# argumentcomputer/lurk-beta

Measured on NVIDIA H100. Metric: Lurk iterations proved/sec (fib rc=100, Nova IVC), higher is better.
Workload: dtype u32x8 (254-bit Montgomery integers)

## Files before the change

### lurk-beta_b200/csrc/curve.cuh

```cuda
#pragma once
#include "field.cuh"

namespace lurk {

template <class F>
struct Affine {
    F x, y;
    LURK_HD bool is_identity() const { return x.is_zero() && y.is_zero(); }
};

template <class F>
LURK_HD F mul_sub_mul(const F &a, const F &b, const F &c, const F &d) {
    WideAcc<typename F::Params> acc;
    acc.clear();
    acc.mul_acc(a, b);
    acc.mul_acc(c.neg(), d);
    return acc.reduce();
}

template <class F>
struct XYZZ {
    F x, y, zz, zzz;

    LURK_HD static XYZZ identity() { XYZZ r; r.x = F::zero(); r.y = F::zero(); r.zz = F::zero(); r.zzz = F::zero(); return r; }
// ... 51 lines not shown
        F ppp = p * pp;
        F q_ = x * pp;
        F x3 = r.sqr() - ppp - q_.dbl();
        y = mul_sub_mul(r, q_ - x3, y, ppp);
        x = x3;
        zz = zz * pp;
        zzz = zzz * ppp;
    }
    LURK_HD void add(const XYZZ &o) {
        if (o.is_identity()) return;
        if (is_identity()) { *this = o; return; }
        F u1 = x * o.zz;
        F u2 = o.x * zz;
        F s1 = y * o.zzz;
        F s2 = o.y * zzz;
        F p = u2 - u1;
        F r = s2 - s1;
        if (p.is_zero()) {
            if (r.is_zero()) *this = dbl(); else *this = identity();
            return;
        }
        F pp = p.sqr();
        F ppp = p * pp;
        F q_ = u1 * pp;
        F x3 = r.sqr() - ppp - q_.dbl();
        y = mul_sub_mul(r, q_ - x3, s1, ppp);
        x = x3;
        zz = zz * o.zz * pp;
        zzz = zzz * o.zzz * ppp;
    }
    LURK_HD Affine<F> to_affine() const {
        Affine<F> a;
        if (is_identity()) { a.x = F::zero(); a.y = F::zero(); return a; }
        F zi = zzz.inv();
        F zz_inv = (zi * zz).sqr();
        a.x = x * zz_inv;
        a.y = y * zi;
        return a;
    }
    LURK_HD XYZZ mul_u32(uint32_t k) const {
        XYZZ acc = identity();
        for (int b = 31; b >= 0; b--) {
            acc = acc.dbl();
            if ((k >> b) & 1) acc.add(*this);
        }
        return acc;
    }
};

struct CurveBn254G1 {
    using Base = Fe<Bn254Fq>; using Scalar = Fe<Bn254Fr>;
    static constexpr int ID = 0; static constexpr bool GEN_X_NEG1 = false;
    LURK_HD static constexpr uint32_t GEN_Y(int i) { constexpr uint32_t t[8] = {2, 0, 0, 0, 0, 0, 0, 0}; return t[i]; }
};
struct CurveGrumpkin {
    using Base = Fe<Bn254Fr>; using Scalar = Fe<Bn254Fq>;
    static constexpr int ID = 1; static constexpr bool GEN_X_NEG1 = false;
    LURK_HD static constexpr uint32_t GEN_Y(int i) {
        constexpr uint32_t t[8] = {0x823f272cu, 0x833fc48du, 0xf1181294u, 0x2d270d45u, 0x06a45d63u, 0xcf135e75u, 0x00000002u, 0x00000000u};
        return t[i];
    }
};
struct CurvePallas {
    using Base = Fe<PallasFp>; using Scalar = Fe<PallasFq>;
    static constexpr int ID = 2; static constexpr bool GEN_X_NEG1 = true;
    LURK_HD static constexpr uint32_t GEN_Y(int i) { constexpr uint32_t t[8] = {2, 0, 0, 0, 0, 0, 0, 0}; return t[i]; }
};
// ... 19 lines not shown
```

### lurk-beta_b200/csrc/field.cuh

```cuda
#pragma once
#include <cstdint>
#include <cstring>

#if defined(__CUDACC__)
#define LURK_HD __host__ __device__ __forceinline__
#define LURK_D __device__ __forceinline__
#else
#define LURK_HD inline
#define LURK_D inline
#endif

#include "field_consts.cuh"

namespace lurk {

namespace cc {
#if defined(__CUDA_ARCH__)
LURK_D uint32_t add_cc(uint32_t a, uint32_t b) { uint32_t r; asm volatile("add.cc.u32 %0, %1, %2;" : "=r"(r) : "r"(a), "r"(b)); return r; }
LURK_D uint32_t addc_cc(uint32_t a, uint32_t b) { uint32_t r; asm volatile("addc.cc.u32 %0, %1, %2;" : "=r"(r) : "r"(a), "r"(b)); return r; }
LURK_D uint32_t addc(uint32_t a, uint32_t b) { uint32_t r; asm volatile("addc.u32 %0, %1, %2;" : "=r"(r) : "r"(a), "r"(b)); return r; }
LURK_D uint32_t sub_cc(uint32_t a, uint32_t b) { uint32_t r; asm volatile("sub.cc.u32 %0, %1, %2;" : "=r"(r) : "r"(a), "r"(b)); return r; }
LURK_D uint32_t subc_cc(uint32_t a, uint32_t b) { uint32_t r; asm volatile("subc.cc.u32 %0, %1, %2;" : "=r"(r) : "r"(a), "r"(b)); return r; }
LURK_D uint32_t subc(uint32_t a, uint32_t b) { uint32_t r; asm volatile("subc.u32 %0, %1, %2;" : "=r"(r) : "r"(a), "r"(b)); return r; }
LURK_D uint32_t mul_lo(uint32_t a, uint32_t b) { uint32_t r; asm volatile("mul.lo.u32 %0, %1, %2;" : "=r"(r) : "r"(a), "r"(b)); return r; }
// ... 202 lines not shown
        uint32_t u[8], w[8];
        Fe x1 = zero(), x2 = zero();
        x1.v[0] = 1;
#pragma unroll
        for (int i = 0; i < 8; i++) { u[i] = v[i]; w[i] = P::MOD(i); }
        auto is_one = [](const uint32_t *a) { uint32_t o = a[0] ^ 1u; for (int i = 1; i < 8; i++) o |= a[i]; return o == 0; };
        auto shr1 = [](uint32_t *a) { for (int i = 0; i < 7; i++) a[i] = (a[i] >> 1) | (a[i + 1] << 31); a[7] >>= 1; };
        auto halve = [&](Fe &x) {
            if (x.v[0] & 1u) {
                x.v[0] = cc::add_cc(x.v[0], P::MOD(0));
                for (int i = 1; i < 7; i++) x.v[i] = cc::addc_cc(x.v[i], P::MOD(i));
                x.v[7] = cc::addc(x.v[7], P::MOD(7));
            }
            shr1(x.v);
        };
        auto sub_raw = [](uint32_t *a, const uint32_t *b) {
            a[0] = cc::sub_cc(a[0], b[0]);
            for (int i = 1; i < 8; i++) a[i] = cc::subc_cc(a[i], b[i]);
            return cc::subc(0, 0);
        };
        auto geq = [](const uint32_t *a, const uint32_t *b) {
            for (int i = 7; i >= 0; i--) { if (a[i] > b[i]) return true; if (a[i] < b[i]) return false; }
            return true;
        };
        while (!is_one(u) && !is_one(w)) {
            while (!(u[0] & 1u)) { shr1(u); halve(x1); }
            while (!(w[0] & 1u)) { shr1(w); halve(x2); }
            if (geq(u, w)) { sub_raw(u, w); x1 = x1 - x2; }
            else { sub_raw(w, u); x2 = x2 - x1; }
        }
        const Fe r3 = rr() * rr();
        return (is_one(u) ? x1 : x2) * r3;
    }
    LURK_HD Fe inv() const {
        uint32_t e[8];
        e[0] = cc::sub_cc(P::MOD(0), 2);
#pragma unroll
        for (int i = 1; i < 8; i++) e[i] = cc::subc_cc(P::MOD(i), 0);
        return pow_raw(e);
    }
};

template <class P, int ROUNDS>
LURK_HD Fe<P> redc17(uint32_t *t) {
    uint32_t r[9];
#pragma unroll
    for (int k = 0; k < 9; k++) r[k] = 0;
#pragma unroll
    for (int i = 0; i < 8; i++) {
        uint32_t mi = t[i] * P::M0;
        Fe<P>::template cmad_mod<0>(t + i, mi);
        r[i] = cc::addc(r[i], 0);
        Fe<P>::template cmad_mod<1>(t + i + 1, mi);
        r[i + 1] = cc::addc(r[i + 1], 0);
    }
    t[8] = cc::add_cc(t[8], r[0]);
#pragma unroll
    for (int k = 1; k < 8; k++) t[8 + k] = cc::addc_cc(t[8 + k], r[k]);
    t[16] = cc::addc(t[16], r[8]);
#pragma unroll
    for (int round = 0; round < ROUNDS; round++) {
        uint32_t d[9];
        d[0] = cc::sub_cc(t[8], P::MOD(0));
#pragma unroll
        for (int k = 1; k < 8; k++) d[k] = cc::subc_cc(t[8 + k], P::MOD(k));
        d[8] = cc::subc_cc(t[16], 0);
// ... 94 lines not shown
```

### lurk-beta_b200/csrc/foldctx_impl.cuh

```cuda
#pragma once
#include "msm_impl.cuh"
#include "poseidon_api.h"
#include "spmv3.cuh"

#include <memory>
#include <string>

namespace lurk {

static constexpr int FOLD_MAX_WORLD = 16;
static constexpr int FOLD_MAX_DEPTH = 4;
static constexpr int FOLD_MAX_SPANS = 4;
static constexpr int FOLD_RO_RATE = 24;
static constexpr int FOLD_W_WINDOW = 17;
static constexpr int FOLD_T_WINDOW = 16;

template <class F>
__global__ void __launch_bounds__(256) cross_term_dev_kernel(const F *__restrict__ az1, const F *__restrict__ bz1, const F *__restrict__ cz1,
                                                             const F *__restrict__ az2, const F *__restrict__ bz2, const F *__restrict__ cz2,
                                                             const F *__restrict__ u1p, const F *__restrict__ u2p, size_t n, F *__restrict__ t) {
    const F u1 = load_fe<F>(u1p), u2 = load_fe<F>(u2p);
    for (size_t i = (size_t)blockIdx.x * blockDim.x + threadIdx.x; i < n; i += (size_t)gridDim.x * blockDim.x) {
        WideAcc<typename F::Params> acc;
        acc.clear();
// ... 227 lines not shown
            const unsigned long long *flag = &a.peers[a.rank]->slot[parity][lane].flag;
            const unsigned long long t0 = globaltimer_ns();
            while (ld_acquire_sys(flag) < seq) {
                if (globaltimer_ns() - t0 > 4000000000ull) { sh_status = 1; break; }
                __nanosleep(200);
            }
        }
        __syncwarp();
        if (lane < a.world) {
            const XchgSlot<Fb> *src = &a.peers[a.rank]->slot[parity][lane];
            const uint4 *q = reinterpret_cast<const uint4 *>(warp == 0 ? &src->w : &src->t);
            uint4 wd[8];
#pragma unroll
            for (int k = 0; k < 8; k++) wd[k] = ld_volatile_u4(q + k);
            const uint32_t *u = reinterpret_cast<const uint32_t *>(wd);
#pragma unroll
            for (int k = 0; k < 8; k++) { pt.x.v[k] = u[k]; pt.y.v[k] = u[8 + k]; pt.zz.v[k] = u[16 + k]; pt.zzz.v[k] = u[24 + k]; }
        }
        int span = 1;
        while (span < a.world) span <<= 1;
#pragma unroll 1
        for (int d = span >> 1; d > 0; d >>= 1) {
            const Pt p2 = shfl_xor_xyzz(pt, d);
            pt.add(p2);
        }
    }
    if (lane == 0) sh_pt[warp] = pt;
    __syncthreads();

    if (tid == 0) {
        const Pt pw = sh_pt[0], pc = sh_pt[1];
        const bool iw = pw.is_identity(), ic = pc.is_identity();
        const Fb zw = iw ? Fb::one() : pw.zzz, zc = ic ? Fb::one() : pc.zzz;
        const Fb inv = (zw * zc).inv_vartime();
        const Fb iwz = inv * zc, icz = inv * zw;
        Fb x = Fb::zero(), y = Fb::zero();
        if (!iw) { const Fb zz_inv = (iwz * pw.zz).sqr(); x = pw.x * zz_inv; y = pw.y * iwz; }
        sh_aff[0] = x; sh_aff[1] = y;
        x = Fb::zero(); y = Fb::zero();
        if (!ic) { const Fb zz_inv = (icz * pc.zz).sqr(); x = pc.x * zz_inv; y = pc.y * icz; }
        sh_aff[2] = x; sh_aff[3] = y;
        sh_inf[0] = iw; sh_inf[1] = ic;
        a.rec->cw_x = sh_aff[0]; a.rec->cw_y = sh_aff[1]; a.rec->ct_x = sh_aff[2]; a.rec->ct_y = sh_aff[3];
        a.rec->cw_inf = iw; a.rec->ct_inf = ic;
        a.rec->status = sh_status;
        a.rec->seq = seq;
    }
    __syncthreads();
    if (a.mode != FOLD_MODE_FOLD || warp != 0) return;

    Fb s = Fb::zero();
    if (lane == 0) s = a.io_tag;
    else if (lane <= a.n_absorb) {
        switch (a.kind[lane - 1]) {
            case FOLD_RO_W_X: s = sh_aff[0]; break;
            case FOLD_RO_W_Y: s = sh_aff[1]; break;
            case FOLD_RO_W_INF: s = sh_inf[0] ? Fb::one() : Fb::zero(); break;
            case FOLD_RO_T_X: s = sh_aff[2]; break;
            case FOLD_RO_T_Y: s = sh_aff[3]; break;
            case FOLD_RO_T_INF: s = sh_inf[1] ? Fb::one() : Fb::zero(); break;
            default: s = load_fe<Fb>(a.step_consts + (lane - 1)); break;
        }
    }
    s = ro_permute_warp<Fb>(a.ro_consts, a.L, s, lane);
    if (lane == 1) {
        a.rec->hash = s;
        const Fb h = s.to_canonical();
// ... 17 lines not shown
__global__ void __launch_bounds__(64) fold_commitments_kernel(XYZZ<typename C::Base> *run_w, XYZZ<typename C::Base> *run_e,
                                                              FoldRecord<typename C::Base, typename C::Scalar> *rec, int init) {
    using Fb = typename C::Base;
    using Fs = typename C::Scalar;
    using Pt = XYZZ<Fb>;
    const int which = threadIdx.x >> 5;
    if (threadIdx.x & 31) return;
    Affine<Fb> q;
    q.x = which == 0 ? rec->cw_x : rec->ct_x;
    q.y = which == 0 ? rec->cw_y : rec->ct_y;
    Pt *run = which == 0 ? run_w : run_e;
    Pt acc;
    if (init) {
        acc = which == 0 ? Pt::from_affine(q) : Pt::identity();
    } else {
        const Fs k = rec->r.to_canonical();
        acc = Pt::identity();
        int top = 255;
        while (top >= 0 && !((k.v[top >> 5] >> (top & 31)) & 1u)) top--;
#pragma unroll 1
        for (int b = top; b >= 0; b--) {
            acc = acc.dbl();
            if ((k.v[b >> 5] >> (b & 31)) & 1u) acc.add_affine(q);
        }
        Pt cur = *run;
        cur.add(acc);
        acc = cur;
    }
    *run = acc;
    Affine<Fb> af;
    af.x = Fb::zero();
    af.y = Fb::zero();
    if (!acc.is_identity()) {
        const Fb zi = acc.zzz.inv_vartime();
        const Fb zz_inv = (zi * acc.zz).sqr();
        af.x = acc.x * zz_inv;
        af.y = acc.y * zi;
    }
    if (which == 0) { rec->uw_x = af.x; rec->uw_y = af.y; rec->uw_inf = acc.is_identity(); }
    else { rec->ue_x = af.x; rec->ue_y = af.y; rec->ue_inf = acc.is_identity(); }
}

struct FoldSpan { uint64_t first, row_elems, stride, rows; };

struct FoldSlotBatch {
    int arity = 0;
    size_t count = 0;
    DevBuf d_offsets;
    DevBuf d_pre[FOLD_MAX_DEPTH];
    void *h_pre[FOLD_MAX_DEPTH] = {nullptr, nullptr, nullptr, nullptr};
    size_t bytes() const { return count * (size_t)(arity ? arity : 1) * 32; }
};

struct FoldConfigHost {
    int curve_id = 0, depth = 2, world = 1, rank = 0;
    uint64_t n_w = 0, n_x = 0, n_rows = 0;
    int latency_sms = 0;
};

struct FoldResultHost {
    uint8_t comm_w[96], comm_t[96], r[32], run_comm_w[96], run_comm_e[96], hash[32];
    int status;
    unsigned long long seq;
};

struct FoldCtxBase {
    virtual ~FoldCtxBase() {}
// ... 29 lines not shown
```

### lurk-beta_b200/csrc/msm_impl.cuh

```cuda
#pragma once
#include "common.cuh"

#include <algorithm>
#include <atomic>
#include <mutex>
#include <thread>

namespace lurk {

static constexpr uint32_t KEY_NONE = 0xffffffffu;

struct MsmPlan {
    int c = 0;
    int nwin = 0;
    uint32_t nb = 0;
    uint32_t total_buckets = 0;
    uint32_t seg = 0;
    uint32_t t1 = 0;
    bool fixed = false;
    uint32_t rwin = 0, K = 0, G = 0, nq = 0, SL = 0, slice = 0;
};
static constexpr uint32_t MSM_MAX_RESULT_POINTS = 512;

inline int fixed_base_window(size_t key_n) {
// ... 83 lines not shown
}

static __global__ void __launch_bounds__(1024) msm_scan_tile_sums_kernel(const uint32_t *__restrict__ counts, uint32_t len, uint32_t *__restrict__ tile_sums) {
    const uint32_t base = blockIdx.x * SCAN_TILE + threadIdx.x * 4;
    uint32_t sum = 0;
#pragma unroll
    for (int k = 0; k < 4; k++) if (base + k < len) sum += counts[base + k];
    uint32_t total;
    block_exclusive_scan_1024(sum, &total);
    if (threadIdx.x == 0) tile_sums[blockIdx.x] = total;
}
static __global__ void __launch_bounds__(1024) msm_scan_tiles_kernel(const uint32_t *__restrict__ tile_sums, uint32_t ntiles, uint32_t *__restrict__ tile_offsets) {
    const uint32_t base = threadIdx.x * 4;
    uint32_t v[4], sum = 0;
#pragma unroll
    for (int k = 0; k < 4; k++) { v[k] = base + k < ntiles ? tile_sums[base + k] : 0; sum += v[k]; }
    uint32_t total;
    uint32_t run = block_exclusive_scan_1024(sum, &total);
#pragma unroll
    for (int k = 0; k < 4; k++) { if (base + k < ntiles) tile_offsets[base + k] = run; run += v[k]; }
    if (threadIdx.x == 0) tile_offsets[ntiles] = total;
}
struct BucketPartials { uint32_t first, count; };
__host__ __device__ __forceinline__ BucketPartials bucket_partials(uint32_t lo, uint32_t hi, uint32_t seg) {
    BucketPartials r{lo / seg + 1, 0};
    if (hi >= lo + 2) {
        const uint32_t last = (hi - 1) / seg;
        if (last >= r.first) r.count = last - r.first + 1;
    }
    return r;
}
static constexpr uint32_t MSM_LONG_PARTIALS = 16;

static __global__ void __launch_bounds__(1024) msm_scan_apply_kernel(const uint32_t *__restrict__ counts, uint32_t len, const uint32_t *__restrict__ tile_offsets,
                                                              uint32_t ntiles, uint32_t *__restrict__ offsets, uint32_t seg = 0,
                                                              uint32_t *long_list = nullptr) {
    const uint32_t base = blockIdx.x * SCAN_TILE + threadIdx.x * 4;
    uint32_t v[4], sum = 0;
#pragma unroll
    for (int k = 0; k < 4; k++) { v[k] = base + k < len ? counts[base + k] : 0; sum += v[k]; }
    uint32_t run = tile_offsets[blockIdx.x] + block_exclusive_scan_1024(sum, nullptr);
#pragma unroll
    for (int k = 0; k < 4; k++) {
        if (base + k < len) {
            offsets[base + k] = run;
            if (long_list && bucket_partials(run, run + v[k], seg).count > MSM_LONG_PARTIALS) long_list[atomicAdd(long_list - 1, 1u)] = base + k;
        }
        run += v[k];
    }
    if (blockIdx.x == 0 && threadIdx.x == 0) offsets[len] = tile_offsets[ntiles];
}

template <class Fs>
__global__ void __launch_bounds__(256) msm_scatter_kernel(const Fs *__restrict__ scalars, const Fs *__restrict__ sub, size_t n, int fmt, int c, int nwin,
                                                          uint32_t key_stride, uint32_t base_stride, const uint32_t *__restrict__ offsets,
                                                          uint32_t *__restrict__ cursor, uint32_t *__restrict__ sorted) {
    size_t i = (size_t)blockIdx.x * blockDim.x + threadIdx.x;
    const bool live = i < n;
    Fs k = Fs::zero();
    if (live) {
        k = load_fe<Fs>(scalars + i);
        if (sub) k = k - load_fe<Fs>(sub + i);
        if (fmt == LURK_FMT_MONTGOMERY) k = k.to_canonical();
    }
    uint32_t carry = 0;
    const uint32_t half = 1u << (c - 1);
    const uint32_t lane = threadIdx.x & 31;
    for (int w = 0; w < nwin; w++) {
        uint32_t raw = window_bits(k.v, w * c, c) + carry;
// ... 102 lines not shown
    PairIn<Fb> r;
    r.p1 = pair_load<Fb, FIRST>(sorted, pts, in);
    r.kind = 0;
    r.p2 = r.p1;
    if (in + 1 < run_end) {
        r.p2 = pair_load<Fb, FIRST>(sorted, pts, in + 1);
        if (r.p1.is_identity()) { r.p1 = r.p2; }
        else if (r.p2.is_identity()) {}
        else if (r.p1.x == r.p2.x) r.kind = (r.p1.y == r.p2.y && !r.p1.y.is_zero()) ? 2 : 3;
        else r.kind = 1;
    }
    return r;
}
template <class Fb>
__device__ __forceinline__ Fb pair_denominator(const PairIn<Fb> &in) {
    if (in.kind == 1) return in.p2.x - in.p1.x;
    if (in.kind == 2) return in.p1.y.dbl();
    return Fb::one();
}

template <class Fb>
__device__ __forceinline__ Fb warp_batch_inverse(const Fb &v) {
    const int lane = threadIdx.x & 31;
    Fb pre = v, suf = v;
#pragma unroll 1
    for (int d = 1; d < 32; d <<= 1) {
        Fb a, b;
#pragma unroll
        for (int i = 0; i < 8; i++) { a.v[i] = __shfl_up_sync(0xffffffffu, pre.v[i], d); b.v[i] = __shfl_down_sync(0xffffffffu, suf.v[i], d); }
        if (lane >= d) pre = pre * a;
        if (lane + d < 32) suf = suf * b;
    }
    Fb inv = Fb::zero();
    if (lane == 31) inv = pre.inv_vartime();
    Fb ep, es, r;
#pragma unroll
    for (int i = 0; i < 8; i++) {
        ep.v[i] = __shfl_up_sync(0xffffffffu, pre.v[i], 1);
        es.v[i] = __shfl_down_sync(0xffffffffu, suf.v[i], 1);
        r.v[i] = __shfl_sync(0xffffffffu, inv.v[i], 31);
    }
    if (lane > 0) r = r * ep;
    if (lane < 31) r = r * es;
    return r;
}

template <class Fb, bool FIRST>
__global__ void __launch_bounds__(128) msm_pair_kernel(const uint32_t *__restrict__ offs_in, const uint32_t *__restrict__ offs_out, uint32_t nbuckets,
                                                       const uint32_t *__restrict__ sorted, const Affine<Fb> *__restrict__ pts_in,
                                                       Affine<Fb> *__restrict__ pts_out) {
    const uint32_t total = offs_out[nbuckets];
    const uint64_t gtid = (uint64_t)blockIdx.x * blockDim.x + threadIdx.x;
    if ((gtid & ~31ull) * PAIR_B >= total) return;
    const uint64_t start64 = gtid * PAIR_B;
    const bool active = start64 < total;
    const uint32_t start = active ? (uint32_t)start64 : 0, end = active ? (uint32_t)min((uint64_t)total, start64 + PAIR_B) : 0;
    uint32_t k = 0;
    if (active) {
        uint32_t lo = 0, hi = nbuckets;
        while (hi - lo > 1) { const uint32_t mid = (lo + hi) >> 1; if (offs_out[mid] <= start) lo = mid; else hi = mid; }
        k = lo;
    }
    Fb pref[PAIR_B];
    Fb run = Fb::one();
    for (uint32_t q = start; q < end; q++) {
        while (offs_out[k + 1] <= q) k++;
        const uint32_t in = offs_in[k] + 2 * (q - offs_out[k]);
        const PairIn<Fb> pi = pair_fetch<Fb, FIRST>(sorted, pts_in, in, offs_in[k + 1]);
        run = run * pair_denominator(pi);
        pref[q - start] = run;
    }
    Fb inv = warp_batch_inverse(run);
    for (uint32_t q = end; q-- > start;) {
        while (offs_out[k] > q) k--;
        const uint32_t in = offs_in[k] + 2 * (q - offs_out[k]);
        const PairIn<Fb> pi = pair_fetch<Fb, FIRST>(sorted, pts_in, in, offs_in[k + 1]);
        const uint32_t j = q - start;
        const Fb den = pair_denominator(pi);
        const Fb inv_d = j ? inv * pref[j - 1] : inv;
        inv = inv * den;
        Affine<Fb> o = pi.p1;
        if (pi.kind == 3) { o.x = Fb::zero(); o.y = Fb::zero(); }
        else if (pi.kind) {
            Fb num;
            if (pi.kind == 1) num = pi.p2.y - pi.p1.y;
            else { const Fb xx = pi.p1.x.sqr(); num = xx.dbl() + xx; }
            const Fb lam = num * inv_d;
            const Fb x3 = lam.sqr() - pi.p1.x - pi.p2.x;
            o.y = lam * (pi.p1.x - x3) - pi.p1.y;
            o.x = x3;
        }
        store_fe(&pts_out[q].x, o.x);
        store_fe(&pts_out[q].y, o.y);
    }
}

static constexpr uint32_t MSM_MERGE_THREADS = 64, MSM_MERGE_LONG_THREADS = 256;
template <class Fb>
__global__ void __launch_bounds__(MSM_MERGE_THREADS) msm_merge_kernel(const uint32_t *__restrict__ offsets, uint32_t nbuckets, uint32_t seg,
                                                                      const XYZZ<Fb> *__restrict__ ppt, XYZZ<Fb> *__restrict__ bucket_acc) {
    const uint32_t b = blockIdx.x * MSM_MERGE_THREADS + threadIdx.x;
    if (b >= nbuckets) return;
    const uint32_t lo = offsets[b], hi = offsets[b + 1];
    const BucketPartials bp = bucket_partials(lo, hi, seg);
    if (bp.count > MSM_LONG_PARTIALS) return;
    XYZZ<Fb> acc = XYZZ<Fb>::identity();
    if (hi > lo) acc = load_xyzz(bucket_acc + b);
    for (uint32_t i = 0; i < bp.count; i++) acc.add(load_xyzz(ppt + bp.first + i));
    store_xyzz(bucket_acc + b, acc);
}

template <class Fb>
__global__ void __launch_bounds__(MSM_MERGE_LONG_THREADS) msm_merge_long_kernel(const uint32_t *__restrict__ offsets, uint32_t seg,
                                                                                const XYZZ<Fb> *__restrict__ ppt, const uint32_t *__restrict__ long_list,
                                                                                XYZZ<Fb> *__restrict__ bucket_acc) {
    __shared__ XYZZ<Fb> sm[MSM_MERGE_LONG_THREADS];
    const uint32_t tid = threadIdx.x, nlong = long_list[-1];
    for (uint32_t i = blockIdx.x; i < nlong; i += gridDim.x) {
        const uint32_t b = long_list[i];
        const BucketPartials bp = bucket_partials(offsets[b], offsets[b + 1], seg);
        XYZZ<Fb> acc = XYZZ<Fb>::identity();
        if (tid == 0) acc = load_xyzz(bucket_acc + b);
        for (uint32_t j = tid; j < bp.count; j += MSM_MERGE_LONG_THREADS) acc.add(load_xyzz(ppt + bp.first + j));
        sm[tid] = acc;
        __syncthreads();
        for (uint32_t stride = MSM_MERGE_LONG_THREADS / 2; stride > 0; stride >>= 1) {
            if (tid < stride) { XYZZ<Fb> x = sm[tid]; x.add(sm[tid + stride]); sm[tid] = x; }
            __syncthreads();
        }
        if (tid == 0) store_xyzz(bucket_acc + b, sm[0]);
        __syncthreads();
    }
}


template <class Fb>
__global__ void __launch_bounds__(128) msm_chunk_kernel(const XYZZ<Fb> *__restrict__ bucket_acc, uint32_t K, uint32_t nchunks_total,
                                                        XYZZ<Fb> *__restrict__ tri_out, XYZZ<Fb> *__restrict__ run_out) {
    const uint32_t g = blockIdx.x * blockDim.x + threadIdx.x;
    if (g >= nchunks_total) return;
    const XYZZ<Fb> *B = bucket_acc + (size_t)g * K;
    XYZZ<Fb> run = XYZZ<Fb>::identity(), tri = XYZZ<Fb>::identity();
    for (int b = (int)K - 1; b >= 0; b--) {
        run.add(load_xyzz(B + b));
        tri.add(run);
    }
    store_xyzz(tri_out + g, tri);
    store_xyzz(run_out + g, run);
}

// ... 165 lines not shown
    cudaEvent_t ev0 = nullptr, ev1 = nullptr;
    float last_accumulate_ms = 0.f;
    unsigned last_launches = 0;
    bool pending = false;
    int pending_fmt = 0, pending_c = 0, pending_nwin = 0;
    bool pending_fixed = false;
    uint32_t pending_nq = 0, pending_K = 0;
    cudaEvent_t done = nullptr;
    cudaStream_t tiny_stream = nullptr;
    const void *d_sub = nullptr;
    const void *d_offset = nullptr;
    cudaEvent_t ev_fork = nullptr, ev_join = nullptr;
};

namespace lurk {

template <class Fb>
void point_to_bytes(const XYZZ<Fb> &p, int fmt, uint8_t out[96]) {
    memset(out, 0, 96);
    if (p.is_identity()) return;
    Affine<Fb> a = p.to_affine();
    Fb one = Fb::one();
    if (fmt == LURK_FMT_CANONICAL) { a.x = a.x.to_canonical(); a.y = a.y.to_canonical(); one = one.to_canonical(); }
    memcpy(out, a.x.v, 32); memcpy(out + 32, a.y.v, 32); memcpy(out + 64, one.v, 32);
}

inline int ctx_check_device(const lurk_msm_ctx *ctx) {
    int dev = -1;
    LURK_CUDA_TRY(cudaGetDevice(&dev));
    if (dev != ctx->device) { set_error("context belongs to device %d but device %d is current", ctx->device, dev); return LURK_ERR_ARG; }
    return LURK_OK;
}

template <class C>
int msm_launch(lurk_msm_ctx *ctx, const void *d_scalars, size_t n, int fmt, cudaStream_t s, bool readback) {
    using Fb = typename C::Base;
    using Fs = typename C::Scalar;
    using Pt = XYZZ<Fb>;
    if (ctx->pending) { set_error("a launch is already pending on this context (call lurk_msm_ctx_finish)"); return LURK_ERR_ARG; }
    LURK_TRY(ctx_check_device(ctx));
    if (!ctx->done) LURK_CUDA_TRY(cudaEventCreateWithFlags(&ctx->done, cudaEventDisableTiming));
    ctx->pending_fmt = fmt;
    ctx->pending_nwin = 0;
    MsmScratch &S = ctx->scratch;
    if (S.result.bytes < sizeof(Pt)) LURK_TRY(S.result.alloc(sizeof(Pt)));
    if (n == 0) {
        if (readback) ctx->pending = true;
        else LURK_CUDA_TRY(cudaMemsetAsync(S.result.p, 0, sizeof(Pt), s));
        return LURK_OK;
    }
    const bool table_pays = !readback || n * (size_t)(Fs::Params::NBITS / std::max(ctx->fixed_c, 1) + 1) >= ((size_t)8 << (std::max(ctx->fixed_c, 1) - 1));
    const bool fixed = ctx->d_table != nullptr && table_pays;
    if (!readback && !fixed) { set_error("device-resident results need the fixed-base table (lurk_msm_ctx_precompute)"); return LURK_ERR_ARG; }
    MsmPlan P = make_plan(n, Fs::Params::NBITS, fixed ? ctx->fixed_c : 0);
    if ((uint64_t)n * (uint64_t)P.nwin >= (1ull << 32)) { set_error("%zu scalars exceed one launch (shard the commitment key)", n); return LURK_ERR_ARG; }
    const uint32_t TB = P.total_buckets;
    const uint32_t ntiles = (TB + SCAN_TILE - 1) / SCAN_TILE;
    const size_t cap = n * (size_t)P.nwin;
    int rounds = 0;
    {
        static const int forced = [] { const char *e = getenv("LURK_MSM_PAIR_ROUNDS"); return e ? atoi(e) : -1; }();
        const size_t avg = cap / TB;
        if (forced >= 0) rounds = forced;
        else if (n >= 8192) rounds = avg >= 12 ? MSM_PAIR_ROUNDS_LONG : (avg >= 5 ? MSM_PAIR_ROUNDS_SHORT : 0);
        if (rounds > 4) rounds = 4;
    }
    size_t cap_final = cap;
    for (int r = 0; r < rounds; r++) cap_final = cap_final / 2 + TB + 1;
    const uint32_t t1 = rounds ? (uint32_t)((cap_final + P.seg - 1) / P.seg) : P.t1;
    const uint32_t t1_alloc = std::max(t1, P.t1);
    const uint32_t max_long = t1 / (MSM_LONG_PARTIALS + 1) + 1;
    {
        auto ensure = [](DevBuf &b, size_t bytes) { return b.bytes >= bytes ? LURK_OK : b.alloc(bytes); };
        LURK_TRY(ensure(S.counts, (((size_t)TB + 1) * 2 + 1 + max_long) * sizeof(uint32_t)));
        LURK_TRY(ensure(S.offsets, ((size_t)TB + 1) * sizeof(uint32_t)));
        LURK_TRY(ensure(S.tiles, ((size_t)ntiles + 1) * 2 * sizeof(uint32_t)));
        LURK_TRY(ensure(S.sorted, n * (size_t)P.nwin * sizeof(uint32_t)));
        LURK_TRY(ensure(S.buckets, (size_t)TB * sizeof(Pt)));
        LURK_TRY(ensure(S.ppt, (size_t)t1_alloc * sizeof(Pt)));
        const size_t nchunks_all = (size_t)P.rwin * P.G;
        LURK_TRY(ensure(S.chunks, nchunks_all * sizeof(Pt)));
        LURK_TRY(ensure(S.chunk_sums, nchunks_all * sizeof(Pt)));
        LURK_TRY(ensure(S.slices, (size_t)P.rwin * P.nq * P.SL * sizeof(Pt)));
        LURK_TRY(ensure(S.wins, MSM_MAX_RESULT_POINTS * sizeof(Pt)));
        if (!S.h_wins) LURK_CUDA_TRY(cudaMallocHost(&S.h_wins, MSM_MAX_RESULT_POINTS * sizeof(Pt)));
    }
    if (ntiles > 4096) { set_error("bucket table too large for the scan"); return LURK_ERR_ARG; }
    uint32_t *counts = S.counts.as<uint32_t>();
    uint32_t *cursor = counts + (TB + 1);
    uint32_t *offsets = S.offsets.as<uint32_t>();
    uint32_t *tile_sums = S.tiles.as<uint32_t>(), *tile_offsets = tile_sums + (ntiles + 1);
    uint32_t *sorted = S.sorted.as<uint32_t>();
    uint32_t *long_list = cursor + (TB + 1) + 1;
    Pt *buckets = S.buckets.as<Pt>();

    LURK_CUDA_TRY(cudaMemsetAsync(counts, 0, (((size_t)TB + 1) * 2 + 1) * sizeof(uint32_t), s));
    const unsigned gs = (unsigned)((n + 255) / 256);
    unsigned launches = 0;
    const uint32_t key_stride = fixed ? 0u : P.nb;
    const uint32_t base_stride = fixed ? (uint32_t)ctx->n : 0u;
    const Affine<Fb> *bases = (const Affine<Fb> *)(fixed ? ctx->d_table : ctx->d_bases);
    const Fs *sub = (!readback && fmt == LURK_FMT_MONTGOMERY) ? (const Fs *)ctx->d_sub : nullptr;
    msm_count_kernel<Fs><<<gs, 256, 0, s>>>((const Fs *)d_scalars, sub, n, fmt, P.c, P.nwin, key_stride, counts);
    msm_scan_tile_sums_kernel<<<ntiles, 1024, 0, s>>>(counts, TB, tile_sums);
    msm_scan_tiles_kernel<<<1, 1024, 0, s>>>(tile_sums, ntiles, tile_offsets);
    msm_scan_apply_kernel<<<ntiles, 1024, 0, s>>>(counts, TB, tile_offsets, ntiles, offsets, P.seg, rounds ? nullptr : long_list);
    msm_scatter_kernel<Fs><<<gs, 256, 0, s>>>((const Fs *)d_scalars, sub, n, fmt, P.c, P.nwin, key_stride, base_stride, offsets, cursor, sorted);
    if (ctx->profile) LURK_CUDA_TRY(cudaEventRecord(ctx->ev0, s));
    const uint32_t *acc_offs = offsets;
    const Affine<Fb> *acc_pts = bases;
    size_t cap_r = cap;
    for (int r = 0; r < rounds; r++) {
        cap_r = cap_r / 2 + TB + 1;
        DevBuf &ob = S.pair_offs[r & 1], &pb = S.pair_pts[r & 1];
        if (ob.bytes < ((size_t)TB + 1) * sizeof(uint32_t)) LURK_TRY(ob.alloc(((size_t)TB + 1) * sizeof(uint32_t)));
        if (pb.bytes < cap_r * sizeof(Affine<Fb>)) LURK_TRY(pb.alloc(cap_r * sizeof(Affine<Fb>)));
        uint32_t *o2 = ob.as<uint32_t>();
        msm_halve_kernel<<<(TB + 256) / 256, 256, 0, s>>>(acc_offs, TB, counts);
        msm_scan_tile_sums_kernel<<<ntiles, 1024, 0, s>>>(counts, TB, tile_sums);
        msm_scan_tiles_kernel<<<1, 1024, 0, s>>>(tile_sums, ntiles, tile_offsets);
        msm_scan_apply_kernel<<<ntiles, 1024, 0, s>>>(counts, TB, tile_offsets, ntiles, o2, P.seg, r == rounds - 1 ? long_list : nullptr);
        const size_t pthreads = (cap_r + PAIR_B - 1) / PAIR_B;
        const unsigned pgrid = (unsigned)((pthreads + 127) / 128);
        if (r == 0) msm_pair_kernel<Fb, true><<<pgrid, 128, 0, s>>>(acc_offs, o2, TB, sorted, acc_pts, pb.as<Affine<Fb>>());
        else msm_pair_kernel<Fb, false><<<pgrid, 128, 0, s>>>(acc_offs, o2, TB, sorted, acc_pts, pb.as<Affine<Fb>>());
        launches += 5;
        acc_offs = o2;
        acc_pts = pb.as<Affine<Fb>>();
    }
    if (rounds)
        msm_accumulate_kernel<Fb, 5, true><<<(t1 + 127) / 128, 128, 0, s>>>(acc_offs, TB, sorted, acc_pts, buckets, S.ppt.as<Pt>(), P.seg, t1);
    else if (fixed)
        msm_accumulate_kernel<Fb, 5><<<(P.t1 + 127) / 128, 128, 0, s>>>(offsets, TB, sorted, bases, buckets, S.ppt.as<Pt>(), P.seg, P.t1);
    else
        msm_accumulate_kernel<Fb, 4><<<(P.t1 + 127) / 128, 128, 0, s>>>(offsets, TB, sorted, bases, buckets, S.ppt.as<Pt>(), P.seg, P.t1);
    if (ctx->profile) LURK_CUDA_TRY(cudaEventRecord(ctx->ev1, s));
    launches += 6;
    msm_merge_long_kernel<Fb><<<std::min<uint32_t>(max_long, 2 * sm_count()), MSM_MERGE_LONG_THREADS, 0, s>>>(acc_offs, P.seg, S.ppt.as<Pt>(),
                                                                                                             long_list, buckets);
    msm_merge_kernel<Fb><<<(TB + MSM_MERGE_THREADS - 1) / MSM_MERGE_THREADS, MSM_MERGE_THREADS, 0, s>>>(acc_offs, TB, P.seg, S.ppt.as<Pt>(), buckets);
    launches += 2;
    const uint32_t nchunks = P.rwin * P.G, nres = P.rwin * P.nq;
    if (nres > MSM_MAX_RESULT_POINTS) { set_error("internal: %u result points", nres); return LURK_ERR_ARG; }
    msm_chunk_kernel<Fb><<<(nchunks + 127) / 128, 128, 0, s>>>(buckets, P.K, nchunks, S.chunks.as<Pt>(), S.chunk_sums.as<Pt>());
    msm_bitsum_kernel<Fb><<<dim3(P.SL, P.nq, P.rwin), 256, 0, s>>>(S.chunks.as<Pt>(), S.chunk_sums.as<Pt>(), P.G, P.slice,
                                                                  P.SL > 1 ? S.slices.as<Pt>() : S.wins.as<Pt>());
    launches += 2;
    if (P.SL > 1) {
        msm_slice_sum_kernel<Fb><<<(nres * 32 + 127) / 128, 128, 0, s>>>(S.slices.as<Pt>(), P.SL, nres, S.wins.as<Pt>());
        launches++;
    }
    if (fixed) {
        cudaStream_t st = ctx->tiny_stream ? ctx->tiny_stream : s;
        if (st != s) {
            LURK_CUDA_TRY(cudaEventRecord(ctx->ev_fork, s));
            LURK_CUDA_TRY(cudaStreamWaitEvent(st, ctx->ev_fork, 0));
        }
        msm_horner_kernel<Fb><<<1, 32, 0, st>>>(S.wins.as<Pt>(), P.nq, P.K, sub ? (const Affine<Fb> *)ctx->d_offset : nullptr, S.result.as<Pt>());
        launches++;
        if (st != s && readback) {
            LURK_CUDA_TRY(cudaEventRecord(ctx->ev_join, st));
            LURK_CUDA_TRY(cudaStreamWaitEvent(s, ctx->ev_join, 0));
        }
    }
    ctx->last_launches = launches;
    LURK_CUDA_TRY(cudaGetLastError());
    if (!readback) return LURK_OK;
    if (fixed) LURK_CUDA_TRY(cudaMemcpyAsync(S.h_wins, S.result.p, sizeof(Pt), cudaMemcpyDeviceToHost, s));
    else LURK_CUDA_TRY(cudaMemcpyAsync(S.h_wins, S.wins.p, (size_t)nres * sizeof(Pt), cudaMemcpyDeviceToHost, s));
    LURK_CUDA_TRY(cudaEventRecord(ctx->done, s));
    ctx->pending = true;
    ctx->pending_c = P.c;
    ctx->pending_nwin = P.nwin;
// ... 105 lines not shown
```

Baseline: 23480.

## Add safegcd field inversion and optional affine batch-inverse MSM accumulation

Adds a Bernstein-Yang style safegcd modular inverse (inv_fast) on 30-bit signed limbs and uses it in place of the exponentiation and vartime binary inversions in to_affine, the fold finalisation and the warp batch inverse. It also adds an optional bucket-accumulation kernel that performs affine additions with a warp-wide batched inversion, plus dynamic segment-length plumbing through the scan and merge kernels. The affine kernel is gated by the LURK_MSM_AFFINE environment variable and stays off by default, so only the new inversion changes the default path. The inversion loop carries divergence and correctness risk on edge inputs.

```diff
diff --git a/lurk-beta_b200/csrc/curve.cuh b/lurk-beta_b200/csrc/curve.cuh
--- a/lurk-beta_b200/csrc/curve.cuh
+++ b/lurk-beta_b200/csrc/curve.cuh
@@ -107,7 +107,7 @@
     LURK_HD Affine<F> to_affine() const {
         Affine<F> a;
         if (is_identity()) { a.x = F::zero(); a.y = F::zero(); return a; }
-        F zi = zzz.inv();
+        F zi = zzz.inv_fast();
         F zz_inv = (zi * zz).sqr();
         a.x = x * zz_inv;
         a.y = y * zi;
diff --git a/lurk-beta_b200/csrc/field.cuh b/lurk-beta_b200/csrc/field.cuh
--- a/lurk-beta_b200/csrc/field.cuh
+++ b/lurk-beta_b200/csrc/field.cuh
@@ -258,6 +258,151 @@
         const Fe r3 = rr() * rr();
         return (is_one(u) ? x1 : x2) * r3;
     }
+    LURK_HD static int ctz32(uint32_t x) {
+#if defined(__CUDA_ARCH__)
+        return __ffs((int)x) - 1;
+#else
+        return __builtin_ctz(x);
+#endif
+    }
+    LURK_HD static int imin(int a, int b) { return a < b ? a : b; }
+    struct S30 { int32_t l[9]; };
+    static constexpr int32_t M30 = 0x3fffffff;
+    LURK_HD static constexpr int32_t mod30(int i) {
+        return (int32_t)(((P::MOD((30 * i) / 32) >> ((30 * i) % 32)) |
+                          ((30 * i) % 32 > 2 && (30 * i) / 32 + 1 < 8 ? P::MOD((30 * i) / 32 + 1) << (32 - (30 * i) % 32) : 0u)) & (uint32_t)M30);
+    }
+    LURK_HD static S30 to_s30(const uint32_t *w) {
+        S30 r;
+        uint64_t acc = 0;
+        int bits = 0, k = 0;
+#pragma unroll
+        for (int i = 0; i < 9; i++) {
+            if (bits < 30 && k < 8) { acc |= (uint64_t)w[k++] << bits; bits += 32; }
+            r.l[i] = (int32_t)(acc & (uint64_t)M30);
+            acc >>= 30;
+            bits -= 30;
+        }
+        return r;
+    }
+    LURK_HD static Fe from_s30(const S30 &s) {
+        Fe r;
+        uint64_t acc = 0;
+        int bits = 0, i = 0;
+#pragma unroll
+        for (int k = 0; k < 8; k++) {
+#pragma unroll
+            for (int t = 0; t < 2; t++)
+                if (bits < 32 && i < 9) { acc |= (uint64_t)(uint32_t)s.l[i++] << bits; bits += 30; }
+            r.v[k] = (uint32_t)acc;
+            acc >>= 32;
+            bits -= 32;
+        }
+        return r;
+    }
+    LURK_HD static void by_update_fg(S30 &f, S30 &g, int32_t u, int32_t v, int32_t q, int32_t r) {
+        int64_t cf = (int64_t)u * f.l[0] + (int64_t)v * g.l[0];
+        int64_t cg = (int64_t)q * f.l[0] + (int64_t)r * g.l[0];
+        cf >>= 30;
+        cg >>= 30;
+#pragma unroll
+        for (int i = 1; i < 9; i++) {
+            cf += (int64_t)u * f.l[i] + (int64_t)v * g.l[i];
+            cg += (int64_t)q * f.l[i] + (int64_t)r * g.l[i];
+            f.l[i - 1] = (int32_t)cf & M30;
+            g.l[i - 1] = (int32_t)cg & M30;
+            cf >>= 30;
+            cg >>= 30;
+        }
+        f.l[8] = (int32_t)cf;
+        g.l[8] = (int32_t)cg;
+    }
+    LURK_HD static void by_normalise(S30 &d) {
+        const int32_t neg = d.l[8] >> 31;
+        int32_t c = 0;
+#pragma unroll
+        for (int i = 0; i < 8; i++) { c += d.l[i] + (mod30(i) & neg); d.l[i] = c & M30; c >>= 30; }
+        d.l[8] += c + (mod30(8) & neg);
+        S30 t;
+        c = 0;
+#pragma unroll
+        for (int i = 0; i < 8; i++) { c += d.l[i] - mod30(i); t.l[i] = c & M30; c >>= 30; }
+        t.l[8] = d.l[8] + c - mod30(8);
+        const bool ge = t.l[8] >= 0;
+#pragma unroll
+        for (int i = 0; i < 9; i++) d.l[i] = ge ? t.l[i] : d.l[i];
+    }
+    LURK_HD static void by_update_de(S30 &d, S30 &e, int32_t u, int32_t v, int32_t q, int32_t r) {
+        const uint32_t md = (((uint32_t)u * (uint32_t)d.l[0] + (uint32_t)v * (uint32_t)e.l[0]) * P::M0) & (uint32_t)M30;
+        const uint32_t me = (((uint32_t)q * (uint32_t)d.l[0] + (uint32_t)r * (uint32_t)e.l[0]) * P::M0) & (uint32_t)M30;
+        int64_t cd = (int64_t)u * d.l[0] + (int64_t)v * e.l[0] + (int64_t)md * mod30(0);
+        int64_t ce = (int64_t)q * d.l[0] + (int64_t)r * e.l[0] + (int64_t)me * mod30(0);
+        cd >>= 30;
+        ce >>= 30;
+#pragma unroll
+        for (int i = 1; i < 9; i++) {
+            cd += (int64_t)u * d.l[i] + (int64_t)v * e.l[i] + (int64_t)md * mod30(i);
+            ce += (int64_t)q * d.l[i] + (int64_t)r * e.l[i] + (int64_t)me * mod30(i);
+            d.l[i - 1] = (int32_t)cd & M30;
+            e.l[i - 1] = (int32_t)ce & M30;
+            cd >>= 30;
+            ce >>= 30;
+        }
+        d.l[8] = (int32_t)cd;
+        e.l[8] = (int32_t)ce;
+        by_normalise(d);
+        by_normalise(e);
+    }
+    LURK_HD Fe inv_fast() const {
+        if (is_zero()) return zero();
+        S30 f, g = to_s30(v), d, e;
+        uint32_t rr_w[8];
+#pragma unroll
+        for (int i = 0; i < 9; i++) { f.l[i] = mod30(i); d.l[i] = 0; }
+#pragma unroll
+        for (int i = 0; i < 8; i++) rr_w[i] = P::RR(i);
+        e = to_s30(rr_w);
+        int32_t eta = -1;
+#pragma unroll 1
+        for (int it = 0; it < 25; it++) {
+            uint32_t fl = (uint32_t)f.l[0] | ((uint32_t)f.l[1] << 30), gl = (uint32_t)g.l[0] | ((uint32_t)g.l[1] << 30);
+            uint32_t u = 1, vv = 0, q = 0, r = 1;
+            int left = 30;
+#pragma unroll 1
+            for (;;) {
+                const int zeros = ctz32(gl | (0xffffffffu << left));
+                gl >>= zeros; u <<= zeros; vv <<= zeros;
+                eta -= zeros;
+                left -= zeros;
+                if (left == 0) break;
+                if (eta < 0) {
+                    eta = -eta;
+                    const uint32_t t0 = fl, t1 = u, t2 = vv;
+                    fl = gl; u = q; vv = r;
+                    gl = 0u - t0; q = 0u - t1; r = 0u - t2;
+                }
+                const int limit = imin(imin(eta + 1, left), 12);
+                uint32_t x = fl;
+                x *= 2u - fl * x;
+                x *= 2u - fl * x;
+                const uint32_t w = (0u - gl * x) & (0xffffffffu >> (32 - limit));
+                gl += fl * w; q += u * w; r += vv * w;
+            }
+            by_update_fg(f, g, (int32_t)u, (int32_t)vv, (int32_t)q, (int32_t)r);
+            by_update_de(d, e, (int32_t)u, (int32_t)vv, (int32_t)q, (int32_t)r);
+            int32_t nz = 0;
+#pragma unroll
+            for (int i = 0; i < 9; i++) nz |= g.l[i];
+            if (!nz) break;
+        }
+        if (f.l[8] < 0) {
+            int32_t c = 0;
+#pragma unroll
+            for (int i = 0; i < 8; i++) { c += mod30(i) - d.l[i]; d.l[i] = c & M30; c >>= 30; }
+            d.l[8] = mod30(8) - d.l[8] + c;
+        }
+        return from_s30(d);
+    }
     LURK_HD Fe inv() const {
         uint32_t e[8];
         e[0] = cc::sub_cc(P::MOD(0), 2);
diff --git a/lurk-beta_b200/csrc/foldctx_impl.cuh b/lurk-beta_b200/csrc/foldctx_impl.cuh
--- a/lurk-beta_b200/csrc/foldctx_impl.cuh
+++ b/lurk-beta_b200/csrc/foldctx_impl.cuh
@@ -283,7 +283,7 @@
         const Pt pw = sh_pt[0], pc = sh_pt[1];
         const bool iw = pw.is_identity(), ic = pc.is_identity();
         const Fb zw = iw ? Fb::one() : pw.zzz, zc = ic ? Fb::one() : pc.zzz;
-        const Fb inv = (zw * zc).inv_vartime();
+        const Fb inv = (zw * zc).inv_fast();
         const Fb iwz = inv * zc, icz = inv * zw;
         Fb x = Fb::zero(), y = Fb::zero();
         if (!iw) { const Fb zz_inv = (iwz * pw.zz).sqr(); x = pw.x * zz_inv; y = pw.y * iwz; }
@@ -367,7 +367,7 @@
     af.x = Fb::zero();
     af.y = Fb::zero();
     if (!acc.is_identity()) {
-        const Fb zi = acc.zzz.inv_vartime();
+        const Fb zi = acc.zzz.inv_fast();
         const Fb zz_inv = (zi * acc.zz).sqr();
         af.x = acc.x * zz_inv;
         af.y = acc.y * zi;
diff --git a/lurk-beta_b200/csrc/msm_impl.cuh b/lurk-beta_b200/csrc/msm_impl.cuh
--- a/lurk-beta_b200/csrc/msm_impl.cuh
+++ b/lurk-beta_b200/csrc/msm_impl.cuh
@@ -139,9 +139,16 @@
 }
 static constexpr uint32_t MSM_LONG_PARTIALS = 16;
 
+__host__ __device__ __forceinline__ uint32_t segment_length(uint32_t total, uint32_t seg_min, uint32_t units) {
+    if (!units) return seg_min;
+    const uint32_t s = (uint32_t)(((uint64_t)total + units - 1) / units);
+    return s > seg_min ? s : seg_min;
+}
+
 static __global__ void __launch_bounds__(1024) msm_scan_apply_kernel(const uint32_t *__restrict__ counts, uint32_t len, const uint32_t *__restrict__ tile_offsets,
-                                                              uint32_t ntiles, uint32_t *__restrict__ offsets, uint32_t seg = 0,
-                                                              uint32_t *long_list = nullptr) {
+                                                              uint32_t ntiles, uint32_t *__restrict__ offsets, uint32_t seg_min = 0,
+                                                              uint32_t *long_list = nullptr, uint32_t units = 0) {
+    const uint32_t seg = long_list ? segment_length(tile_offsets[ntiles], seg_min, units) : seg_min;
     const uint32_t base = blockIdx.x * SCAN_TILE + threadIdx.x * 4;
     uint32_t v[4], sum = 0;
 #pragma unroll
@@ -310,7 +317,7 @@
         if (lane + d < 32) suf = suf * b;
     }
     Fb inv = Fb::zero();
-    if (lane == 31) inv = pre.inv_vartime();
+    if (lane == 31) inv = pre.inv_fast();
     Fb ep, es, r;
 #pragma unroll
     for (int i = 0; i < 8; i++) {
@@ -373,12 +380,154 @@
     }
 }
 
+static constexpr uint32_t MSM_AFF_SEG_MIN = 8;
+enum : uint32_t { AFF_SKIP = 0, AFF_ADD, AFF_DBL, AFF_COPY, AFF_ZERO };
+static constexpr int MSM_AFF_WORDS = 26;
+template <int B>
+constexpr size_t msm_affine_smem() { return (size_t)MSM_AFF_WORDS * 4 * 32 * B; }
+
+template <class Fb>
+__device__ __forceinline__ Fb aff_ld(const uint32_t *p) {
+    Fb r;
+#pragma unroll
+    for (int i = 0; i < 8; i++) r.v[i] = p[i * 32];
+    return r;
+}
+template <class Fb>
+__device__ __forceinline__ void aff_st(uint32_t *p, const Fb &x) {
+#pragma unroll
+    for (int i = 0; i < 8; i++) p[i * 32] = x.v[i];
+}
+template <class Fb>
+__device__ __forceinline__ uint32_t aff_classify(const Affine<Fb> &a, const Affine<Fb> &p, bool active, Fb &den) {
+    den = Fb::one();
+    if (!active || p.is_identity()) return AFF_SKIP;
+    if (a.is_identity()) return AFF_COPY;
+    if (a.x == p.x) {
+        if (a.y == p.y && !a.y.is_zero()) { den = a.y.dbl(); return AFF_DBL; }
+        return AFF_ZERO;
+    }
+    den = p.x - a.x;
+    return AFF_ADD;
+}
+
+template <class Fb, int B>
+__global__ void __launch_bounds__(32) msm_accumulate_affine_kernel(const uint32_t *__restrict__ offsets, uint32_t nbuckets,
+                                                                   const uint32_t *__restrict__ sorted, const Affine<Fb> *__restrict__ bases,
+                                                                   XYZZ<Fb> *__restrict__ bucket_acc, XYZZ<Fb> *__restrict__ ppt,
+                                                                   uint32_t seg_min, uint32_t units) {
+    extern __shared__ uint32_t aff_sm[];
+    const uint32_t lane = threadIdx.x;
+    const uint32_t total = offsets[nbuckets];
+    const uint32_t seg = segment_length(total, seg_min, units);
+    if ((uint64_t)blockIdx.x * 32 * B * seg >= total) return;
+    const uint32_t u0 = (blockIdx.x * 32 + lane) * B;
+    uint32_t *s_key = aff_sm + 24 * 32 * B + lane, *s_rend = s_key + 32 * B;
+    auto acc_x = [&](int j) { return aff_sm + (j * 24) * 32 + lane; };
+    auto acc_y = [&](int j) { return aff_sm + (j * 24 + 8) * 32 + lane; };
+    auto pref = [&](int j) { return aff_sm + (j * 24 + 16) * 32 + lane; };
+#pragma unroll 1
+    for (int j = 0; j < B; j++) {
+        const uint64_t start = (uint64_t)(u0 + j) * seg;
+        uint32_t key = 0, rend = 0;
+        if (start < total) {
+            uint32_t lo = 0, hi = nbuckets;
+            while (hi - lo > 1) {
+                const uint32_t mid = (lo + hi) >> 1;
+                if (offsets[mid] <= (uint32_t)start) lo = mid; else hi = mid;
+            }
+            key = lo;
+            rend = (uint32_t)min((uint64_t)offsets[key + 1], min((uint64_t)total, start + seg));
+        }
+        s_key[j * 32] = key;
+        s_rend[j * 32] = rend;
+        aff_st(acc_x(j), Fb::zero());
+        aff_st(acc_y(j), Fb::zero());
+    }
+    auto fetch = [&](int j, uint32_t s, uint64_t &pos) {
+        pos = (uint64_t)(u0 + j) * seg + s;
+        Affine<Fb> p;
+        p.x = Fb::zero();
+        p.y = Fb::zero();
+        if (pos < total) {
+            const uint32_t e = sorted[pos];
+            p = load_affine(bases + (e & 0x7fffffffu));
+            if (e >> 31) p.y = p.y.neg();
+        }
+        return p;
+    };
+#pragma unroll 1
+    for (uint32_t s = 0; s < seg; s++) {
+        Fb run;
+        uint64_t pos, pos_next;
+        Affine<Fb> p_next = fetch(0, s, pos_next);
+#pragma unroll 1
+        for (int j = 0; j < B; j++) {
+            const Affine<Fb> p = p_next;
+            pos = pos_next;
+            if (j + 1 < B) p_next = fetch(j + 1, s, pos_next);
+            Affine<Fb> a;
+            a.x = aff_ld<Fb>(acc_x(j));
+            a.y = aff_ld<Fb>(acc_y(j));
+            Fb den;
+            aff_classify(a, p, pos < total, den);
+            if (j == 0) run = den;
+            else { aff_st(pref(j), run); run = run * den; }
+        }
+        Fb inv = warp_batch_inverse(run);
+        p_next = fetch(B - 1, s, pos_next);
+#pragma unroll 1
+        for (int j = B - 1; j >= 0; j--) {
+            const Affine<Fb> p = p_next;
+            pos = pos_next;
+            if (j > 0) p_next = fetch(j - 1, s, pos_next);
+            Affine<Fb> a;
+            a.x = aff_ld<Fb>(acc_x(j));
+            a.y = aff_ld<Fb>(acc_y(j));
+            Fb den;
+            const bool active = pos < total;
+            const uint32_t kind = aff_classify(a, p, active, den);
+            Fb inv_d = inv;
+            if (j > 0) { inv_d = inv * aff_ld<Fb>(pref(j)); inv = inv * den; }
+            Fb num = p.y - a.y;
+            if (kind == AFF_DBL) { const Fb xx = a.x.sqr(); num = xx.dbl() + xx; }
+            const Fb lam = num * inv_d;
+            const Fb x3 = lam.sqr() - a.x - p.x;
+            const Fb y3 = lam * (a.x - x3) - a.y;
+            Affine<Fb> r = a;
+            if (kind == AFF_ADD || kind == AFF_DBL) { r.x = x3; r.y = y3; }
+            else if (kind == AFF_COPY) r = p;
+            else if (kind == AFF_ZERO) { r.x = Fb::zero(); r.y = Fb::zero(); }
+            if (active && pos + 1 == s_rend[j * 32]) {
+                uint32_t key = s_key[j * 32];
+                const uint64_t start = (uint64_t)(u0 + j) * seg;
+                XYZZ<Fb> out = XYZZ<Fb>::from_affine(r);
+                if (offsets[key] < start) store_xyzz(ppt + u0 + j, out);
+                else store_xyzz(bucket_acc + key, out);
+                r.x = Fb::zero();
+                r.y = Fb::zero();
+                const uint64_t end = min((uint64_t)total, start + seg);
+                if (pos + 1 < end) {
+                    key++;
+                    while (offsets[key + 1] <= pos + 1) key++;
+                    s_key[j * 32] = key;
+                    s_rend[j * 32] = (uint32_t)min((uint64_t)offsets[key + 1], end);
+                }
+            }
+            aff_st(acc_x(j), r.x);
+            aff_st(acc_y(j), r.y);
+        }
+    }
+}
+
 static constexpr uint32_t MSM_MERGE_THREADS = 64, MSM_MERGE_LONG_THREADS = 256;
 template <class Fb>
-__global__ void __launch_bounds__(MSM_MERGE_THREADS) msm_merge_kernel(const uint32_t *__restrict__ offsets, uint32_t nbuckets, uint32_t seg,
-                                                                      const XYZZ<Fb> *__restrict__ ppt, XYZZ<Fb> *__restrict__ bucket_acc) {
+__global__ void __launch_bounds__(MSM_MERGE_THREADS) msm_merge_kernel(const uint32_t *__restrict__ offsets, uint32_t nbuckets, uint32_t seg_min,
+                                                                      uint32_t units, const XYZZ<Fb> *__restrict__ ppt,
+                                                                      XYZZ<Fb> *__restrict__ bucket_acc) {
     const uint32_t b = blockIdx.x * MSM_MERGE_THREADS + threadIdx.x;
     if (b >= nbuckets) return;
+    const uint32_t seg = segment_length(offsets[nbuckets], seg_min, units);
     const uint32_t lo = offsets[b], hi = offsets[b + 1];
     const BucketPartials bp = bucket_partials(lo, hi, seg);
     if (bp.count > MSM_LONG_PARTIALS) return;
@@ -389,11 +538,13 @@
 }
 
 template <class Fb>
-__global__ void __launch_bounds__(MSM_MERGE_LONG_THREADS) msm_merge_long_kernel(const uint32_t *__restrict__ offsets, uint32_t seg,
+__global__ void __launch_bounds__(MSM_MERGE_LONG_THREADS) msm_merge_long_kernel(const uint32_t *__restrict__ offsets, uint32_t nbuckets,
+                                                                                uint32_t seg_min, uint32_t units,
                                                                                 const XYZZ<Fb> *__restrict__ ppt, const uint32_t *__restrict__ long_list,
                                                                                 XYZZ<Fb> *__restrict__ bucket_acc) {
     __shared__ XYZZ<Fb> sm[MSM_MERGE_LONG_THREADS];
     const uint32_t tid = threadIdx.x, nlong = long_list[-1];
+    const uint32_t seg = segment_length(offsets[nbuckets], seg_min, units);
     for (uint32_t i = blockIdx.x; i < nlong; i += gridDim.x) {
         const uint32_t b = long_list[i];
         const BucketPartials bp = bucket_partials(offsets[b], offsets[b + 1], seg);
@@ -625,6 +776,33 @@
     return LURK_OK;
 }
 
+struct MsmAffineLaunch { int B = 0; unsigned grid = 0; uint32_t units = 0; };
+template <class Fb, int B>
+unsigned msm_affine_grid() {
+    if (msm_affine_smem<B>() > 48 * 1024)
+        cudaFuncSetAttribute(msm_accumulate_affine_kernel<Fb, B>, cudaFuncAttributeMaxDynamicSharedMemorySize, (int)msm_affine_smem<B>());
+    static const unsigned grid = [] {
+        const size_t smem = msm_affine_smem<B>();
+        int per_sm = 0;
+        if (cudaOccupancyMaxActiveBlocksPerMultiprocessor(&per_sm, msm_accumulate_affine_kernel<Fb, B>, 32, smem) != cudaSuccess) per_sm = 0;
+        return (unsigned)std::max(per_sm, 0) * (unsigned)sm_count();
+    }();
+    return grid;
+}
+template <class Fb>
+MsmAffineLaunch msm_affine_launch(size_t cap) {
+    static const char *env = getenv("LURK_MSM_AFFINE");
+    static const bool every_size = env && strncmp(env, "all", 3) == 0;
+    static const int mode = !env ? 0 : every_size ? (env[3] ? atoi(env + 3) : 1) : atoi(env);
+    MsmAffineLaunch a;
+    if (mode == 0) return a;
+    a.B = mode == 16 ? 16 : 8;
+    a.grid = a.B == 16 ? msm_affine_grid<Fb, 16>() : msm_affine_grid<Fb, 8>();
+    a.units = a.grid * 32u * (uint32_t)a.B;
+    if (a.grid == 0 || (!every_size && cap < (size_t)a.units * MSM_AFF_SEG_MIN * 2)) return MsmAffineLaunch{};
+    return a;
+}
+
 template <class C>
 int msm_launch(lurk_msm_ctx *ctx, const void *d_scalars, size_t n, int fmt, cudaStream_t s, bool readback) {
     using Fb = typename C::Base;
@@ -661,8 +839,10 @@
     size_t cap_final = cap;
     for (int r = 0; r < rounds; r++) cap_final = cap_final / 2 + TB + 1;
     const uint32_t t1 = rounds ? (uint32_t)((cap_final + P.seg - 1) / P.seg) : P.t1;
-    const uint32_t t1_alloc = std::max(t1, P.t1);
-    const uint32_t max_long = t1 / (MSM_LONG_PARTIALS + 1) + 1;
+    const MsmAffineLaunch aff = rounds ? MsmAffineLaunch{} : msm_affine_launch<Fb>(cap);
+    const uint32_t seg_min = aff.units ? MSM_AFF_SEG_MIN : P.seg;
+    const uint32_t t1_alloc = std::max({t1, P.t1, aff.units});
+    const uint32_t max_long = t1_alloc / (MSM_LONG_PARTIALS + 1) + 1;
     {
         auto ensure = [](DevBuf &b, size_t bytes) { return b.bytes >= bytes ? LURK_OK : b.alloc(bytes); };
         LURK_TRY(ensure(S.counts, (((size_t)TB + 1) * 2 + 1 + max_long) * sizeof(uint32_t)));
@@ -697,7 +877,7 @@
     msm_count_kernel<Fs><<<gs, 256, 0, s>>>((const Fs *)d_scalars, sub, n, fmt, P.c, P.nwin, key_stride, counts);
     msm_scan_tile_sums_kernel<<<ntiles, 1024, 0, s>>>(counts, TB, tile_sums);
     msm_scan_tiles_kernel<<<1, 1024, 0, s>>>(tile_sums, ntiles, tile_offsets);
-    msm_scan_apply_kernel<<<ntiles, 1024, 0, s>>>(counts, TB, tile_offsets, ntiles, offsets, P.seg, rounds ? nullptr : long_list);
+    msm_scan_apply_kernel<<<ntiles, 1024, 0, s>>>(counts, TB, tile_offsets, ntiles, offsets, seg_min, rounds ? nullptr : long_list, aff.units);
     msm_scatter_kernel<Fs><<<gs, 256, 0, s>>>((const Fs *)d_scalars, sub, n, fmt, P.c, P.nwin, key_stride, base_stride, offsets, cursor, sorted);
     if (ctx->profile) LURK_CUDA_TRY(cudaEventRecord(ctx->ev0, s));
     const uint32_t *acc_offs = offsets;
@@ -723,15 +903,22 @@
     }
     if (rounds)
         msm_accumulate_kernel<Fb, 5, true><<<(t1 + 127) / 128, 128, 0, s>>>(acc_offs, TB, sorted, acc_pts, buckets, S.ppt.as<Pt>(), P.seg, t1);
+    else if (aff.B == 16)
+        msm_accumulate_affine_kernel<Fb, 16><<<aff.grid, 32, msm_affine_smem<16>(), s>>>(offsets, TB, sorted, bases, buckets, S.ppt.as<Pt>(),
+                                                                                        seg_min, aff.units);
+    else if (aff.B == 8)
+        msm_accumulate_affine_kernel<Fb, 8><<<aff.grid, 32, msm_affine_smem<8>(), s>>>(offsets, TB, sorted, bases, buckets, S.ppt.as<Pt>(),
+                                                                                      seg_min, aff.units);
     else if (fixed)
         msm_accumulate_kernel<Fb, 5><<<(P.t1 + 127) / 128, 128, 0, s>>>(offsets, TB, sorted, bases, buckets, S.ppt.as<Pt>(), P.seg, P.t1);
     else
         msm_accumulate_kernel<Fb, 4><<<(P.t1 + 127) / 128, 128, 0, s>>>(offsets, TB, sorted, bases, buckets, S.ppt.as<Pt>(), P.seg, P.t1);
     if (ctx->profile) LURK_CUDA_TRY(cudaEventRecord(ctx->ev1, s));
     launches += 6;
-    msm_merge_long_kernel<Fb><<<std::min<uint32_t>(max_long, 2 * sm_count()), MSM_MERGE_LONG_THREADS, 0, s>>>(acc_offs, P.seg, S.ppt.as<Pt>(),
-                                                                                                             long_list, buckets);
-    msm_merge_kernel<Fb><<<(TB + MSM_MERGE_THREADS - 1) / MSM_MERGE_THREADS, MSM_MERGE_THREADS, 0, s>>>(acc_offs, TB, P.seg, S.ppt.as<Pt>(), buckets);
+    msm_merge_long_kernel<Fb><<<std::min<uint32_t>(max_long, 2 * sm_count()), MSM_MERGE_LONG_THREADS, 0, s>>>(acc_offs, TB, seg_min, aff.units,
+                                                                                                             S.ppt.as<Pt>(), long_list, buckets);
+    msm_merge_kernel<Fb><<<(TB + MSM_MERGE_THREADS - 1) / MSM_MERGE_THREADS, MSM_MERGE_THREADS, 0, s>>>(acc_offs, TB, seg_min, aff.units,
+                                                                                                        S.ppt.as<Pt>(), buckets);
     launches += 2;
     const uint32_t nchunks = P.rwin * P.G, nres = P.rwin * P.nq;
     if (nres > MSM_MAX_RESULT_POINTS) { set_error("internal: %u result points", nres); return LURK_ERR_ARG; }
```

New measurement: 23440 (median of 6 runs). Within noise of the previous version (-0.2%).
